# yulong314/multi_camera_calibration

Hardware: AMD Instinct MI355X
Metric: corner residual+Jacobian evals/sec + ms/LM-iter; RMS reproj-err vs ref (higher is better)
Workload: dtype f64; 1 GPU; config4: 4 omnidirectional cameras, 1000 synthetic 11x8-board views (BASELINE.json configs[3]), one Gauss-Newton step per 'step'; model=omnidirectional, cameras=4, views=1000, edges=3958, params=6018, parallelism=photo-sharded x1, transport=none, state_dtype=f32, jacobian_dtype=f64

## Files before the change

multi_camera_calibration_amd/csrc/mcc_api.cpp:

```cpp
#include <hip/hip_runtime.h>
#include <rccl/rccl.h>

#include <algorithm>
#include <chrono>
#include <cmath>
#include <cstdio>
#include <cstring>
#include <mutex>
#include <numeric>
#include <string>
#include <vector>

#include "../../include/mcc.h"
#include "mcc_internal.h"

using mcc::State;

namespace {

thread_local std::string g_err;

int fail(int code, const std::string& msg) {
    g_err = msg;
    return code;
// ... 99 lines not shown
void tilt_matrix(double tx, double ty, double M[9]) {
    const double cx = std::cos(tx), sx = std::sin(tx), cy = std::cos(ty), sy = std::sin(ty);
    const double rx[9] = {1, 0, 0, 0, cx, sx, 0, -sx, cx};
    const double ry[9] = {cy, 0, -sy, 0, 1, 0, sy, 0, cy};
    double rxy[9];
    for (int i = 0; i < 3; ++i)
        for (int j = 0; j < 3; ++j) {
            double s = 0;
            for (int k = 0; k < 3; ++k) s += ry[3 * i + k] * rx[3 * k + j];
            rxy[3 * i + j] = s;
        }
    const double pz[9] = {rxy[8], 0, -rxy[2], 0, rxy[8], -rxy[5], 0, 0, 1};
    for (int i = 0; i < 3; ++i)
        for (int j = 0; j < 3; ++j) {
            double s = 0;
            for (int k = 0; k < 3; ++k) s += pz[3 * i + k] * rxy[3 * k + j];
            M[3 * i + j] = s;
        }
}

}

struct mcc_problem {
    int model = 0, C = 0, V = 0, E = 0, nd = 0, m = 0, P = 0, device = 0;
    long long corners = 0;
    bool rational = false;
    int prism = 0;
    int has_back = 0;
    int max_epp = 1, nblk = 0, n_items = 0, n_pairs = 0, n_norm_chunks = 0;
    size_t n_pair_doubles = 0;
    int n_pgroups = 0, max_gpairs = 0, max_gcon = 0, max_gedges = 0;
    size_t photo_shmem = 0;
    int use_group = 1;
    size_t group_shmem = 0;
    int group_lanes = 32;
    static constexpr int kFusedMaxM = 30;
    int fused = 0, group_size = 1, n_groups = 1;
    int max_cpp = 1;
    hipStream_t stream = nullptr;

    std::vector<int> dev2ref_edge;
    std::vector<long long> dev2ref_corner;
    std::vector<int> edge_n_dev;

    DevBuf<float> obj_x, obj_y, obj_z, img_u, img_v, x, xerr, K, D, xi, cam_rt, cam_pose, resid, edge_sum, corner_err;
    DevBuf<long long> stamps;
    DevBuf<double> ds_rt, Y, pairprod, zp, gp_tot, item_out, packed, dg, delta, photo_norm, alpha, contrib, gsum, W;
    DevBuf<double> erec, echain, eh;
    DevBuf<double> tilt;
    DevBuf<double> ssinv;
    DevBuf<int> ssinv_ok;
    DevBuf<int> photo_ptr, photo_corner, edge_gblock, block_items, edge_photo, counter, cnt, cnt_blk;
    DevBuf<int> pgrp_ptr, pgrp_edge, gpair_ptr, gcon_ptr;
    DevBuf<int> prep_ptr, prep_edge;
    bool poison = false;
    int poison_level = 0;
    bool peer_push = true;
    int schur_one_level = 0;
    int n_prep = 0, prep_lanes = 1;
    bool warm = false;
    hipStream_t side = nullptr;
    double* sinv = nullptr;
    double* prev2 = nullptr;
    int prev_stride = 0;
    unsigned* wsync = nullptr;
    double* xsol = nullptr;
    bool helper_refine = false;
    int helper_early = 0;
    int inv_la = 0;
    DevBuf<long long> warm_stats;
    int warm_poison = 0;
    long long warm_wait_ticks = 1000000000LL, warm_idle_ticks = 4000000000LL, warm_delay_ticks = 0;
    long long spare_delay_ticks = 0;
    bool small_stats = false;
    bool gfold = false;
    int fold_direct = 0;
    int fold_dyn = 0;
    int fold_first = 0;
    DevBuf<int> fold_ticket;
    int max_item_slots = 0;
    DevBuf<double> fnorm, fiv;
    int fault_photo = -1;
    DevBuf<unsigned char> edge_lphoto;
    DevBuf<unsigned> gcon;
    DevBuf<int4> edge_info, items, gpairs;
    DevBuf<State> state;
    State* h_state = nullptr;
    float* h_x = nullptr;
    int packed_len = 0, ntri = 0;

    static constexpr int kGraphSteps = 8;
    static constexpr int kGraphSizes = 7;
    hipGraphExec_t gexec[kGraphSizes] = {};
    hipGraphExec_t lin_graph = nullptr;
    int lin_graph_n = 0;
    DevBuf<float> xsave;
    DevBuf<double> ysave, zpsave;
    int graph_sizes = kGraphSizes;
    bool use_graph = true;
    bool stepping = false;

    ncclComm_t comm = nullptr;
    int nranks = 1, rank = 0;

    static constexpr int kPeerMaxRanks = MCC_PEER_MAX_RANKS;
    unsigned long long* inbox = nullptr;
// ... 37 lines not shown
                        p->helper_refine && !copy_prev ? 1 : 0, p->xsol, p->helper_early,
                        p->stamps.p ? p->stamps.p + p->stamps.n - 64 : nullptr, p->inv_la};
}

mcc::PeerCtx peer_ctx(mcc_problem* p, bool on) {
    mcc::PeerCtx pc{};
    if (!on) return pc;
    pc.inbox = p->inbox;
    pc.peers = p->peers_dev;
    pc.nranks = p->peer_n;
    pc.rank = p->rank;
    pc.Lc = p->packed_len;
    pc.timeout = p->peer_timeout;
    return pc;
}

void drop_graphs(mcc_problem* p) {
    for (auto& g : p->gexec)
        if (g) { (void)hipGraphExecDestroy(g); g = nullptr; }
    if (p->lin_graph) { (void)hipGraphExecDestroy(p->lin_graph); p->lin_graph = nullptr; }
}

int enqueue_step(mcc_problem* p, int do_update, float* resid_dev, bool lin_only = false) {
    using namespace mcc;
    const bool tim = p->timing && p->ev_used + 2 <= (int)p->ev_lin.size();
    const bool swarm = p->ssinv.p && (p->peer_on || !p->comm);
    if (p->poison) {
        for (auto* b : {&p->contrib, &p->gsum, &p->item_out, &p->pairprod, &p->packed, &p->ssinv})
            if (b->p && b->n && !(swarm && b == &p->packed) && !(p->fused && b == &p->ssinv))
                HIPCHK(hipMemsetAsync(b->p, 0xFF, sizeof(double) * b->n, p->stream));
        if (swarm && !p->fused) HIPCHK(hipMemsetAsync(p->ssinv_ok.p, 0xFF, 2 * sizeof(int), p->stream));
        for (auto* b : {&p->erec, &p->echain, &p->eh})
            if (b->p && b->n) HIPCHK(hipMemsetAsync(b->p, 0xFF, sizeof(double) * b->n, p->stream));
        if (p->poison_level > 1 && p->dg.p) HIPCHK(hipMemsetAsync(p->dg.p, 0xFF, sizeof(double) * p->dg.n, p->stream));
    }
    if (tim) HIPCHK(hipEventRecord(p->ev_step[p->ev_used], p->stream));
    if (tim) HIPCHK(hipEventRecord(p->ev_lin[p->ev_used], p->stream));
    LinArgs la{};
    la.state = p->state.p;
    la.photo_ptr = p->photo_ptr.p;
    la.photo_corner = p->photo_corner.p;
    la.max_cpp = p->max_cpp;
    la.edge_info = p->edge_info.p;
    la.obj_x = p->obj_x.p; la.obj_y = p->obj_y.p; la.obj_z = p->obj_z.p;
    la.img_u = p->img_u.p; la.img_v = p->img_v.p;
    la.x = p->x.p;
    la.K = p->K.p; la.D = p->D.p; la.xi = p->xi.p; la.tilt = p->tilt.p;
    la.cam_rt = p->cam_rt.p; la.ds_rt = p->ds_rt.p;
    la.nd = p->nd; la.global_dim = p->m;
    la.n_cams = p->C; la.has_back = p->has_back;
    la.Y = p->Y.p; la.zp = p->zp.p;
    la.pgrp_ptr = p->pgrp_ptr.p; la.pgrp_edge = p->pgrp_edge.p; la.edge_lphoto = p->edge_lphoto.p; la.gpair_ptr = p->gpair_ptr.p; la.gpairs = p->gpairs.p;
    la.gcon_ptr = p->gcon_ptr.p; la.gcon = p->gcon.p; la.pairprod = p->pairprod.p;
    la.prep_ptr = p->prep_ptr.p; la.prep_edge = p->prep_edge.p; la.n_prep = p->n_prep; la.prep_lanes = p->prep_lanes;
    la.n_pgroups = p->n_pgroups; la.max_gpairs = p->max_gpairs; la.max_gcon = p->max_gcon; la.max_gedges = p->max_gedges;
    la.gp_tot = p->gp_tot.p;
    la.resid = resid_dev;
    la.gblock = p->edge_gblock.p;
    la.dg = p->dg.p;
    la.photo_norm = p->photo_norm.p;
    la.stamps = p->stamps.p;
    la.fault_photo = p->fault_photo;
    const bool lwarm = swarm && (do_update || !p->fused);
    la.ssinv = lwarm ? p->ssinv.p : nullptr;
    la.ssinv_ok = lwarm ? p->ssinv_ok.p : nullptr;
    la.spare_wait = p->warm_wait_ticks;
    la.spare_delay = p->spare_delay_ticks;
    const bool peer = p->peer_on;
    const bool rccl = p->comm != nullptr && !peer;
    la.fused = p->fused;
    la.group_size = p->group_size; la.n_groups = p->n_groups;
    la.rank = p->rank; la.fuse_solve = rccl ? 0 : 1;
    la.peer = peer_ctx(p, peer && p->fused);
    la.contrib = p->contrib.p; la.gsum = p->gsum.p; la.cnt = p->cnt.p; la.packed = p->packed.p; la.W = p->W.p;
    la.solve = solve_ctx(p, do_update);
    la.solve.stamps = nullptr;
    la.n_edges = p->E; la.n_photos = p->V;
    la.erec = p->erec.p; la.echain = p->echain.p; la.eh = p->eh.p;
    SchurArgs sa{};
    const bool split = rccl || p->m > 30;
    if (!p->fused) {
        sa.state = p->state.p;
        sa.items = p->items.p;
        sa.pairprod = p->pairprod.p;
        sa.item_out = p->item_out.p;
        sa.n_items = p->n_items;
        sa.photo_norm = p->photo_norm.p; sa.n_photos = p->V;
        sa.counter = p->counter.p;
        sa.cnt_blk = p->cnt_blk.p;
        sa.nblk = p->nblk;
        sa.block_items = p->block_items.p;
        sa.packed = p->packed.p;
        sa.m = p->m; sa.rank = p->rank; sa.fuse_solve = split ? 0 : 1;
        sa.one_level = p->schur_one_level;
        sa.prev2 = p->warm && do_update && !p->comm && !p->peer_on ? p->prev2 : nullptr;
        sa.prev_stride = p->prev_stride;
        sa.wpub = sa.prev2 && p->helper_refine ? p->wsync : nullptr;
        sa.wpub_early = p->helper_early;
        sa.ssinv = swarm ? p->ssinv.p : nullptr;
        sa.ssinv_ok = swarm ? p->ssinv_ok.p : nullptr;
        sa.peer = peer_ctx(p, peer && !split);
        sa.solve = solve_ctx(p, do_update);
        sa.stamps = p->stamps.p ? p->stamps.p + mcc::kStampStride * (size_t)std::max(p->V, 1) : nullptr;
    }
    const bool fold = p->gfold && !lin_only;
    if (fold) {
// ... 493 lines not shown
    p->group_size = std::max(1, (int)std::ceil(std::sqrt((double)std::max(V, 1))));
    p->n_groups = (std::max(V, 1) + p->group_size - 1) / p->group_size;

    std::vector<float> cam_rt(6 * C, 0.f);
    if (d->model == MCC_MODEL_DOUBLESIDE) {
        for (int c = 0; c < C; ++c) {
            double R[9], r[3];
            for (int i = 0; i < 3; ++i)
                for (int j = 0; j < 3; ++j) R[i * 3 + j] = d->cam_pose[16 * c + i * 4 + j];
            host_rodrigues_m2v(R, r);
            for (int i = 0; i < 3; ++i) { cam_rt[6 * c + i] = (float)r[i]; cam_rt[6 * c + 3 + i] = d->cam_pose[16 * c + i * 4 + 3]; }
        }
    }
    double ds_rt[6] = {0, 0, 0, 0, 0, 0};
    if (d->ds_pose && d->model == MCC_MODEL_PINHOLE) {
        double R[9];
        for (int i = 0; i < 3; ++i)
            for (int j = 0; j < 3; ++j) R[i * 3 + j] = d->ds_pose[i * 4 + j];
        host_rodrigues_m2v(R, ds_rt);
        for (int i = 0; i < 3; ++i) ds_rt[3 + i] = d->ds_pose[i * 4 + 3];
    }
    std::vector<double> alpha(4096);
    for (size_t k = 0; k < alpha.size(); ++k) alpha[k] = std::pow(0.95, (double)k + 1.0);

    HIPC(p->obj_x.upload(ox.data(), ncorner)); HIPC(p->obj_y.upload(oy.data(), ncorner));
    HIPC(p->obj_z.upload(oz.data(), ncorner));
    HIPC(p->img_u.upload(iu.data(), ncorner)); HIPC(p->img_v.upload(iv.data(), ncorner));
    HIPC(p->edge_info.upload(info.data(), E));
    HIPC(p->edge_gblock.upload(gblock.data(), E));
    HIPC(p->edge_photo.upload(ephoto.data(), E));
    HIPC(p->photo_ptr.upload(photo_ptr.data(), V + 1));
    HIPC(p->photo_corner.upload(photo_corner.data(), V + 1));
    HIPC(p->K.upload(d->K, 9 * C));
    HIPC(p->D.upload(d->D, (size_t)d->nd * C));
    std::vector<float> xi(C, 0.f);
    if (d->xi) std::copy(d->xi, d->xi + C, xi.begin());
    HIPC(p->xi.upload(xi.data(), C));
    HIPC(p->cam_rt.upload(cam_rt.data(), 6 * C));
    std::vector<float> cp(16 * C, 0.f);
    if (d->cam_pose) std::copy(d->cam_pose, d->cam_pose + 16 * C, cp.begin());
    HIPC(p->cam_pose.upload(cp.data(), 16 * C));
    HIPC(p->ds_rt.upload(ds_rt, 6));
    HIPC(p->alpha.upload(alpha.data(), alpha.size()));
    HIPC(p->pgrp_ptr.upload(pgrp_ptr.data(), pgrp_ptr.size()));
    {
        std::vector<int> pgrp_edge(pgrp_ptr.size());
        for (size_t g = 0; g < pgrp_ptr.size(); ++g) pgrp_edge[g] = photo_ptr[pgrp_ptr[g]];
        HIPC(p->pgrp_edge.upload(pgrp_edge.data(), pgrp_edge.size()));
        std::vector<unsigned char> lph(std::max(E, 1), 0);
        for (size_t g = 0; g + 1 < pgrp_ptr.size(); ++g)
            for (int v = pgrp_ptr[g]; v < pgrp_ptr[g + 1]; ++v)
                for (int e = photo_ptr[v]; e < photo_ptr[v + 1]; ++e) lph[e] = (unsigned char)(v - pgrp_ptr[g]);
        HIPC(p->edge_lphoto.upload(lph.data(), lph.size()));
    }
    if (!p->fused && !p->use_group) {
        if (const char* f = std::getenv("MCC_PREP_LANES")) p->prep_lanes = std::atoi(f) == 4 ? 4 : 1;
        std::vector<int> pp(1, 0);
        for (int v = 0; v < V;) {
            int w = v, edges = 0;
            while (w < V && w - v < mcc::kPrepPhotos &&
                   (w == v || edges + (photo_ptr[w + 1] - photo_ptr[w]) <= mcc::kPrepEdges)) {
                edges += photo_ptr[w + 1] - photo_ptr[w];
                ++w;
            }
            pp.push_back(w);
            v = w;
        }
        std::vector<int> pe(pp.size());
        for (size_t g = 0; g < pp.size(); ++g) pe[g] = photo_ptr[pp[g]];
        p->n_prep = (int)pp.size() - 1;
        HIPC(p->prep_ptr.upload(pp.data(), pp.size()));
        HIPC(p->prep_edge.upload(pe.data(), pe.size()));
    }
    HIPC(p->gpair_ptr.upload(gpair_ptr.data(), gpair_ptr.size()));
    HIPC(p->gpairs.upload(gpairs.data(), gpairs.size()));
    HIPC(p->gcon_ptr.upload(gcon_ptr.data(), gcon_ptr.size()));
    HIPC(p->gcon.upload(gcon.data(), gcon.size()));
    HIPC(p->items.upload(items.data(), items.size()));
    HIPC(p->block_items.upload(block_items.data(), block_items.size()));
    HIPC(p->x.alloc(p->P)); HIPC(p->xerr.alloc(p->P));
    HIPC(p->Y.alloc(36 * (size_t)E));
    HIPC(p->pairprod.alloc(p->fused ? 0 : p->n_pair_doubles));
    const bool use_split = !p->fused && !p->use_group;
    HIPC(p->erec.alloc(use_split ? 12 * (size_t)E : 0));
    HIPC(p->echain.alloc(use_split ? 54 * (size_t)E : 0));
    HIPC(p->eh.alloc(use_split ? 90 * (size_t)E : 0));
    HIPC(p->zp.alloc(6 * (size_t)V));
    HIPC(p->gp_tot.alloc(6 * (size_t)V));
    HIPC(p->item_out.alloc(48 * (size_t)(items.size() + p->n_norm_chunks + 24)));
    HIPC(hipMemset(p->item_out.p, 0, sizeof(double) * p->item_out.n));
    HIPC(p->counter.alloc(1));
    HIPC(hipMemset(p->counter.p, 0, sizeof(int)));
    HIPC(p->cnt_blk.alloc(p->nblk));
    HIPC(hipMemset(p->cnt_blk.p, 0, sizeof(int) * std::max(p->nblk, 1)));
    p->ntri = p->m * (p->m + 1) / 2;
    p->packed_len = p->ntri + 2 * p->m + 2;
    HIPC(p->packed.alloc(p->packed_len));
    HIPC(p->dg.alloc(p->m)); HIPC(p->delta.alloc(p->P));
    HIPC(p->photo_norm.alloc(2 * (size_t)V));
    if (p->fused) {
        const size_t lcp = (size_t)((p->packed_len + 1) & ~1);
        HIPC(p->contrib.alloc(lcp * std::max(V, 1)));
        HIPC(p->gsum.alloc(lcp * p->n_groups));
        HIPC(p->W.alloc((size_t)6 * p->m * std::max(V, 1)));
        HIPC(p->cnt.alloc(p->n_groups + 1));
        HIPC(hipMemset(p->cnt.p, 0, sizeof(int) * (p->n_groups + 1)));
// ... 82 lines not shown
        HIPC(hipMalloc((void**)&p->sinv, M * M * sizeof(double)));
        p->prev_stride = (p->ntri + p->m + 1) & ~1;
        HIPC(hipExtMallocWithFlags((void**)&p->prev2, 2 * (size_t)p->prev_stride * sizeof(double), hipDeviceMallocUncached));
        if (int r = reset_prev2(p, true)) return bail(r);
        HIPC(hipExtMallocWithFlags((void**)&p->wsync, 8 * sizeof(unsigned), hipDeviceMallocUncached));
        HIPC(hipMemset(p->wsync, 0, 8 * sizeof(unsigned)));
        HIPC(hipExtMallocWithFlags((void**)&p->xsol, 128 * sizeof(double), hipDeviceMallocUncached));
        HIPC(hipMemset(p->xsol, 0, 128 * sizeof(double)));
        if (!p->warm_stats.p) HIPC(p->warm_stats.alloc(5));
        HIPC(hipMemset(p->warm_stats.p, 0, 5 * sizeof(long long)));
        HIPC(stream_pool().take(d->device, &p->side, true));
    }
#undef HIPC
    (void)rc;
    *out = p;
    return MCC_OK;
}

void mcc_destroy(mcc_problem* p) {
    if (!p) return;
    (void)hipSetDevice(p->device);
    const bool side_drained = p->side && hipStreamSynchronize(p->side) == hipSuccess;
    const bool drained = p->stream && hipStreamSynchronize(p->stream) == hipSuccess;
    if (p->sinv) (void)hipFree(p->sinv);
    if (p->prev2) (void)hipFree(p->prev2);
    if (p->wsync) (void)hipFree(p->wsync);
    if (p->xsol) (void)hipFree(p->xsol);
    p->warm_stats.release();
    drop_graphs(p);
    p->xsave.release(); p->ysave.release(); p->zpsave.release();
    for (auto e : p->ev_lin) (void)hipEventDestroy(e);
    for (auto e : p->ev_step) (void)hipEventDestroy(e);
    for (auto e : p->ev_opt) if (e) (void)hipEventDestroy(e);
    for (auto e : p->ev_x) (void)hipEventDestroy(e);
    for (auto e : p->ev_marks) (void)hipEventDestroy(e);
    for (auto e : p->ev_win) if (e) (void)hipEventDestroy(e);
    if (p->comm) (void)ncclCommDestroy(p->comm);
    for (void* m : p->peer_mapped) (void)hipIpcCloseMemHandle(m);
    if (p->peers_dev) (void)hipFree(p->peers_dev);
    if (p->peer_scratch) (void)hipFree(p->peer_scratch);
    if (p->inbox) (void)hipFree(p->inbox);
    p->obj_x.release(); p->obj_y.release(); p->obj_z.release(); p->img_u.release(); p->img_v.release();
    p->x.release(); p->xerr.release(); p->K.release(); p->D.release(); p->xi.release(); p->cam_rt.release();
    p->cam_pose.release(); p->resid.release(); p->edge_sum.release(); p->corner_err.release(); p->stamps.release();
    p->contrib.release(); p->gsum.release(); p->cnt.release(); p->W.release();
    p->ds_rt.release(); p->Y.release(); p->pairprod.release(); p->zp.release();
    p->erec.release(); p->echain.release(); p->eh.release(); p->tilt.release(); p->fnorm.release(); p->fiv.release();
    p->fold_ticket.release(); p->ssinv.release(); p->ssinv_ok.release();
    p->gp_tot.release(); p->item_out.release(); p->packed.release(); p->dg.release(); p->delta.release();
    p->photo_norm.release(); p->alpha.release();
    p->photo_ptr.release(); p->photo_corner.release(); p->edge_gblock.release(); p->block_items.release(); p->counter.release(); p->cnt_blk.release();
    p->edge_photo.release(); p->edge_info.release(); p->items.release(); p->gpairs.release();
    p->prep_ptr.release(); p->prep_edge.release();
    p->pgrp_ptr.release(); p->pgrp_edge.release(); p->edge_lphoto.release(); p->gpair_ptr.release(); p->gcon_ptr.release(); p->gcon.release();
    p->state.release();
    if (p->h_state) (void)hipHostFree(p->h_state);
    if (p->h_x) (void)hipHostFree(p->h_x);
    if (drained) stream_pool().give(p->device, p->stream);
    else if (p->stream) (void)hipStreamDestroy(p->stream);
    if (side_drained) stream_pool().give(p->device, p->side, true);
    else if (p->side) (void)hipStreamDestroy(p->side);
    delete p;
}

int mcc_set_params(mcc_problem* p, const float* x, int n) {
    if (!p || !x || n != p->P) return fail(MCC_EINVAL, "mcc_set_params: size mismatch");
    HIPCHK(hipSetDevice(p->device));
    HIPCHK(hipStreamSynchronize(p->stream));
    HIPCHK(hipMemcpy(p->x.p, x, sizeof(float) * n, hipMemcpyHostToDevice));
    int rc = set_state(p, 1, 0, 0, 0.0);
    if (rc) return rc;
    const int zero = 0;
    HIPCHK(hipMemcpy(&p->state.p->pending, &zero, sizeof(int), hipMemcpyHostToDevice));
    return MCC_OK;
}

int mcc_get_params(mcc_problem* p, float* x, int n) {
    if (!p || !x || n != p->P) return fail(MCC_EINVAL, "mcc_get_params: size mismatch");
    HIPCHK(hipSetDevice(p->device));
    int rc = flush_pending(p);
    if (rc) return rc;
    HIPCHK(hipStreamSynchronize(p->stream));
    HIPCHK(hipMemcpy(x, p->x.p, sizeof(float) * n, hipMemcpyDeviceToHost));
    return MCC_OK;
}

int mcc_linearize_solve(mcc_problem* p, double* delta, double* jte) {
    if (!p) return fail(MCC_EINVAL, "null problem");
    HIPCHK(hipSetDevice(p->device));
    int rc = flush_pending(p);
    if (rc) return rc;
    if ((rc = set_state(p, 0, 0, 0, 0.0))) return rc;
    if ((rc = enqueue_step(p, 0, nullptr))) return rc;
    if ((rc = enqueue_backsub(p, 0))) return rc;
    if ((rc = read_state(p))) return rc;
    if ((rc = check_state_error(p))) return rc;
    if (delta) HIPCHK(hipMemcpy(delta, p->delta.p, sizeof(double) * p->P, hipMemcpyDeviceToHost));
    if (jte) {
        std::vector<double> pk(p->packed_len), gp(6 * (size_t)p->V);
        HIPCHK(hipMemcpy(pk.data(), p->packed.p, sizeof(double) * p->packed_len, hipMemcpyDeviceToHost));
        if (p->V) HIPCHK(hipMemcpy(gp.data(), p->gp_tot.p, sizeof(double) * 6 * p->V, hipMemcpyDeviceToHost));
        for (int i = 0; i < p->m; ++i) jte[i] = pk[p->ntri + p->m + i];
        for (int i = 0; i < 6 * p->V; ++i) jte[p->m + i] = gp[i];
    }
    return MCC_OK;
}
// ... 584 lines not shown
```

multi_camera_calibration_amd/csrc/mcc_group.hpp:

```cpp


template <int MODEL, bool BACK, int L, int GW = 28>
__device__ __forceinline__ void group_prologue(const double* ph, const double* ct, const double* sds, int side,
                                               int sub, double* S, double* P, double* Gb) {
    const double* R1 = ph;
    const double* Jr1 = ph + 9;
    const double* T1 = ph + 18;
    const double* R2 = ct;
    const double* Jl2 = ct + 9;
    const double* T2 = ct + 18;
    double* X = S;
    double* W = S + 15;
    for (int e = sub; e < 12; e += L) {
        if (e < 9) {
            const int i = e / 3, j = e % 3;
            X[e] = dot3_nc(R2[i * 3], R1[j], R2[i * 3 + 1], R1[3 + j], R2[i * 3 + 2], R1[6 + j]);
        } else {
            const int i = e - 9;
            const double q = dot3_nc(R2[i * 3], T1[0], R2[i * 3 + 1], T1[1], R2[i * 3 + 2], T1[2]);
            X[12 + i] = q;
            X[9 + i] = add_nc(q, T2[i]);
        }
    }
    wave_sync_lds();
// ... 552 lines not shown
        fold_final_reset(la, src, have, useiv);
        return;
    }
    __syncthreads();
    if (a.peer.nranks > 0) {
        if (!peer_exchange(a.peer, st, a.packed)) {
            fold_final_reset(la, src, have, useiv);
            return;
        }
        for (int t = tid; t < ntri + m; t += nt) {
            const double v = a.packed[t];
            if (t < ntri) {
                int i, j;
                packed_ij(t, m, i, j);
                S[i * m + j] = v;
                S[j * m + i] = v;
            } else {
                r[t - ntri] = v;
            }
        }
        if (tid < 2) norms[tid] = a.packed[ntri + 2 * m + tid];
        __syncthreads();
    }
    SSTAMP(srow, 3, 0);
    SolveCtx sc = a.solve;
    sc.stamps = srow;
    solve_global<false>(sc, S, r, norms[0], norms[1], nullptr, ivok ? Iv : nullptr);
    SSTAMP(srow, 7, 0);
    fold_final_reset(la, src, have, useiv);
}
template <int NT>
__device__ __forceinline__ void fold_final(const LinArgs& la) {
    if (NT == 512 && la.fold_direct) {
        fold_final_direct(la);
        return;
    }
    constexpr int UM = kSchurOneLevelLoads * 256 / NT;
    const int n = 48 * la.fold_parts + (la.fsa.ssinv != nullptr ? la.fsa.m * la.fsa.m + 1 : 0);
    if (n <= UM / 2 * NT) fold_final_u<UM / 2>(la);
    else fold_final_u<UM>(la);
}

#ifndef MCC_GROUP_PAIR_THREADS
#define MCC_GROUP_PAIR_THREADS 256
#endif
#ifndef MCC_GROUP_OCC
#define MCC_GROUP_OCC 2
#endif
template <int MODEL, bool RATIONAL, int PRISM, bool BACK, int L>
__device__ __forceinline__ bool group_body(const LinArgs& a, const int grp) {
    constexpr int NT = kGroupRound * L, EPW = 64 / L;
    State* st = a.state;
    const int tid = threadIdx.x, lane = tid & 63, wave = tid >> 6;
    const int done = st->done, pending = st->pending;
    const double alpha_prev = st->alpha;
    const int p0 = a.pgrp_ptr[grp], np = a.pgrp_ptr[grp + 1] - p0;
    const int ge0 = a.pgrp_edge[grp], gne = a.pgrp_edge[grp + 1] - ge0;
    const int q0 = a.gpair_ptr[grp], nq = a.gpair_ptr[grp + 1] - q0;
    const int c0 = a.gcon_ptr[grp], nc = a.gcon_ptr[grp + 1] - c0;
    if (done) return false;
    long long* stp = a.stamps ? a.stamps + kStampStride * (size_t)grp : nullptr;
    SSTAMP(stp, 0, 0);
    const int C = a.n_cams, m = a.global_dim;
    extern __shared__ __attribute__((aligned(16))) double smem[];
    const GroupLayout GL = group_layout(gne, C, nq, nc);
    double* rec = smem + GL.rec;
    double* s27 = smem + GL.s27;
    double* sLi = smem + GL.sLi;
    double* sv = smem + GL.sv;
    double* sph = smem + GL.sph;
    double* sxn = smem + GL.sxn;
    double* spart = smem + GL.spart;
    double* sdg = smem + GL.sdg;
    double* ctab = smem + GL.ctab;
    double* ktab = smem + GL.ktab;
    double* sds = smem + GL.sds;
    double* sP = smem + GL.sP;
    double* sGb = smem + GL.sGb;
    int* ibase = reinterpret_cast<int*>(smem + GL.ndoubles);
    int4* sInfo = reinterpret_cast<int4*>(ibase + GL.iInfo);
    int* sgb = ibase + GL.iGb;
    int* seq = ibase + GL.iEq;
    int* sph0 = ibase + GL.iPh;
    int4* spq = reinterpret_cast<int4*>(ibase + GL.iPq);
    unsigned* scn = reinterpret_cast<unsigned*>(ibase + GL.iCn);
    float(*sC)[kGChunk][EPW] = reinterpret_cast<float(*)[kGChunk][EPW]>(smem + GL.sU + wave * (5 * kGChunk * EPW / 2));
    GroupChain* sCH = reinterpret_cast<GroupChain*>(smem + GL.sU + wave * (5 * kGChunk * EPW / 2));
    static_assert(EPW * sizeof(GroupChain) <= 5 * kGChunk * EPW * sizeof(float), "k_group chain union");

    const int g = lane % EPW, sub = lane / EPW;
    auto stage = [&](int eoff, int cc0, int cn) {
        constexpr int PER = kGChunk / L;
        float v[PER][5];
        int sb = sub;
        asm volatile("" : "+v"(sb));
#pragma unroll
        for (int u = 0; u < PER; ++u) {
            const int i = sb + L * u;
            const unsigned c = (unsigned)(eoff + cc0 + (i < cn ? i : 0));
            v[u][0] = a.obj_x[c];
            v[u][1] = a.obj_y[c];
            v[u][2] = a.obj_z[c];
            v[u][3] = a.img_u[c];
            v[u][4] = a.img_v[c];
        }
#pragma unroll
        for (int u = 0; u < PER; ++u) {
            const int i = sb + L * u;
            if (i < cn) {
#pragma unroll
                for (int f = 0; f < 5; ++f) sC[f][i][g] = v[u][f];
            }
        }
    };

    constexpr int CAM0 = NT / 2, DST = CAM0 + 63;
    double om2[3] = {0.0, 0.0, 0.0}, T2[3] = {0.0, 0.0, 0.0};
    {
        {
            const int le = wave * EPW + g;
            const int4 info = le < gne ? a.edge_info[ge0 + le] : make_int4(0, 0, 0, 0);
            if (le < gne) stage(info.z, 0, min(info.w, kGChunk));
        }
        for (int t = tid; t < gne; t += NT) {
            sInfo[t] = a.edge_info[ge0 + t];
            sgb[t] = a.gblock[ge0 + t];
            seq[t] = a.edge_lphoto[ge0 + t];
        }
        if (tid <= np) sph0[tid] = a.photo_ptr[p0 + tid] - ge0;
        for (int t = tid; t < nq; t += NT) spq[t] = a.gpairs[q0 + t];
        for (int t = tid; t < nc; t += NT) scn[t] = a.gcon[c0 + t];
        for (int t = tid; t < m; t += NT) sdg[t] = a.dg[t];
        if (tid >= CAM0 && tid < CAM0 + C) {
            const int c = tid - CAM0;
            if (MODEL == MCC_MODEL_DOUBLESIDE) {
#pragma unroll
                for (int k = 0; k < 3; ++k) { om2[k] = a.cam_rt[6 * c + k]; T2[k] = a.cam_rt[6 * c + 3 + k]; }
            } else if (c == 0) {
#pragma unroll
                for (int k = 0; k < 3; ++k) { om2[k] = 0.0; T2[k] = 0.0; }
            } else {
#pragma unroll
                for (int k = 0; k < 3; ++k) { om2[k] = a.x[6 * (c - 1) + k]; T2[k] = a.x[6 * (c - 1) + 3 + k]; }
            }
            double* kt = ktab + kGIntr * c;
            const float* Kc = a.K + 9 * c;
            kt[0] = Kc[0]; kt[1] = Kc[4]; kt[2] = Kc[2]; kt[3] = Kc[5]; kt[4] = Kc[1];
            kt[5] = MODEL == MCC_MODEL_OMNI ? (double)a.xi[c] : 0.0;
            const int nd = a.nd;
#pragma unroll
            for (int q = 0; q < 12; ++q) kt[6 + q] = q < nd ? (double)a.D[nd * c + q] : 0.0;
            if (PRISM == 2)
#pragma unroll
                for (int q = 0; q < 9; ++q) kt[18 + q] = a.tilt[9 * c + q];
        } else if (BACK && tid == DST) {
            if (MODEL == MCC_MODEL_DOUBLESIDE) {
#pragma unroll
                for (int k = 0; k < 3; ++k) { om2[k] = a.x[k]; T2[k] = a.x[3 + k]; }
            } else {
#pragma unroll
                for (int k = 0; k < 3; ++k) { om2[k] = a.ds_rt[k]; T2[k] = a.ds_rt[3 + k]; }
            }
        }
    }
    float xo = 0.f;
    double zk = 0.0;
    const int pq = (tid - 192) / 6, pk = (tid - 192) % 6;
    const bool ptask = tid >= 192 && pq < np;
    double2 pn0 = make_double2(0.0, 0.0);
    if (ptask) {
        xo = a.x[m + 6 * (size_t)(p0 + pq) + pk];
        if (pending) zk = a.zp[6 * (size_t)(p0 + pq) + pk];
        else if (a.fold && pk == 0) pn0 = *reinterpret_cast<const double2*>(a.photo_norm + 2 * (size_t)(p0 + pq));
    }
    double y0[6];
    int gb0 = -1;
    if (pending && tid < 6 * gne) {
        const int le = tid / 6, k = tid % 6;
        gb0 = a.gblock[ge0 + le];
        const double* Ye = a.Y + 36 * (size_t)(ge0 + le);
#pragma unroll
        for (int i = 0; i < 6; ++i) y0[i] = Ye[6 * i + k];
    }
    __syncthreads();
    SSTAMP(stp, 1, 0);
    if (pending) {
        for (int t = tid; t < 6 * gne; t += NT) {
            const int le = t / 6, k = t % 6;
            int gbl = gb0;
            double y[6];
            if (t == tid) {
#pragma unroll
                for (int i = 0; i < 6; ++i) y[i] = y0[i];
            } else {
                gbl = sgb[le];
                const double* Ye = a.Y + 36 * (size_t)(ge0 + le);
#pragma unroll
                for (int i = 0; i < 6; ++i) y[i] = Ye[6 * i + k];
            }
            const double* d = sdg + 6 * (gbl < 0 ? 0 : gbl);
            double sk = 0.0;
#pragma unroll
            for (int i = 0; i < 6; ++i) sk += y[i] * d[i];
            spart[6 * le + k] = gbl < 0 ? 0.0 : sk;
        }
    }
    __syncthreads();
    if (tid >= CAM0 && tid < CAM0 + C) {
        const int c = tid - CAM0;
        Rot r2;
        rodrigues_v2m(om2, r2);
        double J[9];
        so3_jac(om2, r2, +1.0, J);
        double* ct = ctab + 24 * c;
#pragma unroll
        for (int k = 0; k < 9; ++k) { ct[k] = r2.R[k]; ct[9 + k] = J[k]; }
#pragma unroll
        for (int k = 0; k < 3; ++k) ct[18 + k] = T2[k];
    } else if (BACK && tid == DST) {
        Rot rd;
        rodrigues_v2m(om2, rd);
        double J[9];
        so3_jac(om2, rd, -1.0, J);
#pragma unroll
        for (int k = 0; k < 9; ++k) { sds[k] = rd.R[k]; sds[9 + k] = J[k]; }
#pragma unroll
        for (int k = 0; k < 3; ++k) sds[18 + k] = T2[k];
    }
    if (ptask) {
        float xn = xo;
        double Gk = 0.0;
        if (pending) {
            double t = zk;
            for (int le = sph0[pq]; le < sph0[pq + 1]; ++le) t -= spart[6 * le + pk];
            const float G = (float)(alpha_prev * t);
            xn = xo + G;
            a.x[m + 6 * (size_t)(p0 + pq) + pk] = xn;
            Gk = (double)G;
        }
        sxn[16 * pq + pk] = (double)xn;
        sxn[16 * pq + 8 + pk] = Gk;
    }
    wave_sync_lds();
    if (ptask && pk == 0) {
        const double* xs = sxn + 16 * pq;
        if (pending) {
            double g2 = 0.0, x2 = 0.0;
#pragma unroll
            for (int q = 0; q < 6; ++q) {
                g2 += xs[8 + q] * xs[8 + q];
                x2 += xs[q] * xs[q];
            }
            a.photo_norm[2 * (size_t)(p0 + pq)] = g2;
            a.photo_norm[2 * (size_t)(p0 + pq) + 1] = x2;
            pn0 = make_double2(g2, x2);
        }
        if (a.fold) {
            sxn[16 * pq + 6] = pn0.x;
            sxn[16 * pq + 7] = pn0.y;
        }
        const double om1[3] = {xs[0], xs[1], xs[2]};
        Rot r1;
        rodrigues_v2m(om1, r1);
        double* ph = sph + 24 * pq;
        so3_jac(om1, r1, -1.0, ph + 9);
#pragma unroll
        for (int k = 0; k < 9; ++k) ph[k] = r1.R[k];
#pragma unroll
        for (int k = 0; k < 3; ++k) ph[18 + k] = xs[3 + k];
    }
    __syncthreads();
    SSTAMP(stp, 2, 0);

    for (int rb = 0; rb < gne; rb += kGroupRound) {
        const int es = wave * EPW + g, le = rb + es;
        const bool ev = le < gne;
        const int4 info = ev ? sInfo[le] : make_int4(0, 0, 0, 0);
        const int cam = info.x;
        double* P = sP + kGRecP * es;
        double* Gbe = sGb + 56 * es;
        if (rb > 0 && ev) stage(info.z, 0, min(info.w, kGChunk));
        if (ev) {
            group_prologue<MODEL, BACK, L>(sph + 24 * seq[le], ctab + 24 * cam, sds, info.y, sub, rec + kGRec * le, P, Gbe);
            const double* kt = ktab + kGIntr * cam;
            for (int k = sub; k < (PRISM == 2 ? 27 : 18); k += L) P[12 + k] = kt[k];
        }
        wave_sync_lds();
        if (rb == 0) SSTAMP(stp, 3, 0);
        double acc[32];
#pragma unroll
        for (int q = 0; q < 32; ++q) acc[q] = 0.0;
        const int nn = info.w;
        for (int cc0 = 0;; cc0 += kGChunk) {
            if (cc0 >= nn) break;
            const int cn = min(nn - cc0, kGChunk);
            if (cc0 > 0) {
                wave_sync_lds();
                stage(info.z, cc0, cn);
                wave_sync_lds();
            }
#pragma unroll 1
            for (int i = sub; i < cn; i += L) {
                int po = 0;
                asm volatile("" : "+v"(po));
                const double* Pq = P + po;
                double R[9], T[3], kd[12];
#pragma unroll
                for (int q = 0; q < 9; ++q) R[q] = Pq[q];
#pragma unroll
                for (int q = 0; q < 3; ++q) T[q] = Pq[9 + q];
#pragma unroll
                for (int q = 0; q < 12; ++q) kd[q] = Pq[18 + q];
                const double fx = Pq[12], fy = Pq[13], cx = Pq[14], cy = Pq[15], sk = Pq[16], xi = Pq[17];
                const double X = sC[0][i][g], Y = sC[1][i][g], Z = sC[2][i][g];
                const float ou = sC[3][i][g], ov = sC[4][i][g];
                double Yr[3], D[6];
                float u, v;
                if (MODEL == MCC_MODEL_OMNI)
                    omni_corner(R, T, kd, fx, fy, cx, cy, sk, xi, X, Y, Z, Yr, u, v, D);
                else
                    pinhole_corner<RATIONAL, PRISM>(R, T, kd, fx, fy, cx, cy, X, Y, Z, Yr, u, v, D, Pq + 30);
                const float euf = ou - u, evf = ov - v;
                if (a.resid) {
                    const size_t c = (size_t)info.z + cc0 + i;
                    a.resid[2 * c] = euf;
// ... 439 lines not shown
```

multi_camera_calibration_amd/csrc/mcc_internal.h:

```cpp
#pragma once
#include <hip/hip_runtime.h>

#include "../../include/mcc.h"

namespace mcc {

constexpr int kStampStride = 32;
constexpr int kSchurStampStride = 16;

struct State {
    int iter;
    int done;
    int crit_type;
    int max_count;
    double eps;
    double change;
    double alpha;
    double cam_normG2, cam_normX2;
    int error;
    int pending;
    unsigned int epoch;
    long long xchg_ticks;
    unsigned int spare_ack;
};
// ... 54 lines not shown
    const int4* edge_info;
    const float* obj_x; const float* obj_y; const float* obj_z;
    const float* img_u; const float* img_v;
    float* x;
    const float* K; const float* D; const float* xi;
    const double* tilt;
    const float* cam_rt;
    const double* ds_rt;
    int nd, global_dim, n_cams, has_back;
    double* Y;
    const int* pgrp_ptr;
    const int* pgrp_edge;
    const unsigned char* edge_lphoto;
    const int* gpair_ptr;
    const int4* gpairs;
    const int* gcon_ptr;
    const unsigned* gcon;
    double* pairprod;
    int n_pgroups, max_gpairs, max_gcon, max_gedges;
    double* zp;
    double* gp_tot;
    float* resid;
    const int* gblock;
    const double* dg;
    double* photo_norm;
    long long* stamps;
    int fused, group_size, n_groups, rank, fuse_solve;
    double* contrib;
    double* gsum;
    int* cnt;
    double* packed;
    double* W;
    SolveCtx solve;
    PeerCtx peer;
    int n_edges, n_photos;
    double* erec;
    double* echain;
    double* eh;
    const int* prep_ptr;
    const int* prep_edge;
    int n_prep, prep_lanes;
    int fault_photo;
    int fold_first;
    double* ssinv;
    int* ssinv_ok;
    long long spare_wait, spare_delay;
    int fold, fold_parts;
    int fold_direct;
    int fold_dyn;
    int* fold_ticket;
    SchurArgs fsa;
    double* fnorm;
    double* fiv;
};
constexpr long long kFoldEmpty = -1LL;

constexpr int kItemSingle = 256;
constexpr int kPhotoGroup = 8;
constexpr int kPhotoGroupEdges = 64;
constexpr int kGroupRound = 16;
__host__ __device__ inline size_t photo_lds_doubles(int gne) {
    return (size_t)64 * gne + (size_t)70 * kPhotoGroup;
}
__host__ __device__ inline size_t photo_lds_bytes(int gne, int npairs, int ncon) {
    return photo_lds_doubles(gne) * 8 + 4 * (size_t)((2 * gne + 3) & ~3) + 16 * (size_t)npairs + 4 * (size_t)ncon;
}

constexpr int kGChunk = 96;
constexpr int kGIntr = 28;
constexpr int kGRecP = 40;
constexpr int kGRec = 92;

struct GroupLayout {
    int rec, s27, sLi, sv, sph, sxn, spart, sdg, ctab, ktab, sds, sP, sGb, sU, ndoubles;
    int iInfo, iGb, iEq, iPh, iPq, iCn, nints;
};
__host__ __device__ inline GroupLayout group_layout(int gne, int C, int nq, int nc) {
    GroupLayout L;
    L.rec = 0;
    L.s27 = L.rec + kGRec * gne;
    L.sLi = L.s27 + 28 * kPhotoGroup;
    L.sv = L.sLi + 36 * kPhotoGroup;
    L.sph = L.sv + 6 * kPhotoGroup;
    L.sxn = L.sph + 24 * kPhotoGroup;
    L.spart = L.sxn + 16 * kPhotoGroup;
    L.sdg = L.spart + 6 * gne;
    L.ctab = L.sdg + 128;
    L.ktab = L.ctab + 24 * C;
    L.sds = L.ktab + kGIntr * C;
    L.sP = L.sds + 32;
    L.sGb = L.sP + kGRecP * kGroupRound;
    L.sU = L.sGb + 56 * kGroupRound;
    L.ndoubles = L.sU + 4 * (5 * kGChunk * 4 / 2);
    L.ndoubles = (L.ndoubles + 1) & ~1;
    L.iInfo = 0;
    L.iGb = L.iInfo + 4 * gne;
    L.iEq = L.iGb + gne;
    L.iPh = L.iEq + gne;
    L.iPq = (L.iPh + kPhotoGroup + 1 + 3) & ~3;
    L.iCn = L.iPq + 4 * nq;
    L.nints = L.iCn + nc;
    return L;
}
__host__ __device__ inline size_t group_lds_bytes(int gne, int C, int nq, int nc) {
    const GroupLayout L = group_layout(gne, C, nq, nc);
    return (size_t)L.ndoubles * 8 + (size_t)L.nints * 4;
}

constexpr int kPrepEdges = 16;
constexpr int kPrepPhotos = kPhotoGroup;
struct PrepLayout {
    int tab, S, sdg, sxn, scam, ndoubles;
    int iInfo, iGb, iPh, nints;
// ... 109 lines not shown
```

Measured before the change: 13.04 billion corner evals/s.

## Pack per-group headers and camera intrinsics on host, batch group-kernel prologue loads

Precomputes a per-group header (ranges, photo offsets, first-round edge info, gblock and local-photo indices) and a per-camera intrinsics table on the host at setup. The group linearization kernel then reads these through wave-uniform, predicated register loads instead of chains of dependent scattered loads. Those loads are issued together with the first corner-chunk staging load, and the LDS store of that chunk is deferred until after the pending-update phase so its latency overlaps other work. This shortens the kernel prologue latency, at the cost of extra setup buffers, more register pressure, and intrinsics that are frozen at setup time.

New measurement: 13.74 billion corner evals/s, median of 6. 1.05x the previous value.

```diff
diff --git a/multi_camera_calibration_amd/csrc/mcc_api.cpp b/multi_camera_calibration_amd/csrc/mcc_api.cpp
--- a/multi_camera_calibration_amd/csrc/mcc_api.cpp
+++ b/multi_camera_calibration_amd/csrc/mcc_api.cpp
@@ -175,6 +175,8 @@
     DevBuf<int> ssinv_ok;
     DevBuf<int> photo_ptr, photo_corner, edge_gblock, block_items, edge_photo, counter, cnt, cnt_blk;
     DevBuf<int> pgrp_ptr, pgrp_edge, gpair_ptr, gcon_ptr;
+    DevBuf<int> ghdr;
+    DevBuf<double> kintr;
     DevBuf<int> prep_ptr, prep_edge;
     bool poison = false;
     int poison_level = 0;
@@ -318,6 +320,7 @@
     la.Y = p->Y.p; la.zp = p->zp.p;
     la.pgrp_ptr = p->pgrp_ptr.p; la.pgrp_edge = p->pgrp_edge.p; la.edge_lphoto = p->edge_lphoto.p; la.gpair_ptr = p->gpair_ptr.p; la.gpairs = p->gpairs.p;
     la.gcon_ptr = p->gcon_ptr.p; la.gcon = p->gcon.p; la.pairprod = p->pairprod.p;
+    la.ghdr = p->ghdr.p; la.kintr = p->kintr.p;
     la.prep_ptr = p->prep_ptr.p; la.prep_edge = p->prep_edge.p; la.n_prep = p->n_prep; la.prep_lanes = p->prep_lanes;
     la.n_pgroups = p->n_pgroups; la.max_gpairs = p->max_gpairs; la.max_gcon = p->max_gcon; la.max_gedges = p->max_gedges;
     la.gp_tot = p->gp_tot.p;
@@ -917,6 +920,33 @@
             for (int v = pgrp_ptr[g]; v < pgrp_ptr[g + 1]; ++v)
                 for (int e = photo_ptr[v]; e < photo_ptr[v + 1]; ++e) lph[e] = (unsigned char)(v - pgrp_ptr[g]);
         HIPC(p->edge_lphoto.upload(lph.data(), lph.size()));
+        std::vector<int> hdr((size_t)mcc::kGHdrInts * std::max(NG, 1), 0);
+        for (int g = 0; g < NG; ++g) {
+            int* h = hdr.data() + (size_t)mcc::kGHdrInts * g;
+            const int p0 = pgrp_ptr[g], np = pgrp_ptr[g + 1] - p0, ge0 = photo_ptr[p0], gne = photo_ptr[p0 + np] - ge0;
+            h[0] = p0; h[1] = np; h[2] = ge0; h[3] = gne;
+            h[4] = gpair_ptr[g]; h[5] = gpair_ptr[g + 1] - gpair_ptr[g];
+            h[6] = gcon_ptr[g]; h[7] = gcon_ptr[g + 1] - gcon_ptr[g];
+            for (int q = 0; q <= mcc::kPhotoGroup; ++q) h[mcc::kGHdrPhoto + q] = photo_ptr[p0 + std::min(q, np)] - ge0;
+            for (int le = 0; le < std::min(gne, mcc::kGroupRound); ++le) {
+                const int4 f = info[ge0 + le];
+                int* hi = h + mcc::kGHdrInfo + 4 * le;
+                hi[0] = f.x; hi[1] = f.y; hi[2] = f.z; hi[3] = f.w;
+                h[mcc::kGHdrGb + le] = gblock[ge0 + le];
+                h[mcc::kGHdrEq + le] = lph[ge0 + le];
+            }
+        }
+        HIPC(p->ghdr.upload(hdr.data(), hdr.size()));
+        std::vector<double> kin((size_t)mcc::kGIntr * C, 0.0);
+        for (int c = 0; c < C; ++c) {
+            double* kt = kin.data() + (size_t)mcc::kGIntr * c;
+            const float* Kc = d->K + 9 * c;
+            kt[0] = Kc[0]; kt[1] = Kc[4]; kt[2] = Kc[2]; kt[3] = Kc[5]; kt[4] = Kc[1];
+            kt[5] = d->model == MCC_MODEL_OMNI ? (double)xi[c] : 0.0;
+            for (int q = 0; q < 12; ++q) kt[6 + q] = q < d->nd ? (double)d->D[d->nd * c + q] : 0.0;
+            if (p->prism == 2) tilt_matrix(d->D[14 * c + 12], d->D[14 * c + 13], kt + 18);
+        }
+        HIPC(p->kintr.upload(kin.data(), kin.size()));
     }
     if (!p->fused && !p->use_group) {
         if (const char* f = std::getenv("MCC_PREP_LANES")) p->prep_lanes = std::atoi(f) == 4 ? 4 : 1;
@@ -1105,6 +1135,7 @@
     p->photo_ptr.release(); p->photo_corner.release(); p->edge_gblock.release(); p->block_items.release(); p->counter.release(); p->cnt_blk.release();
     p->edge_photo.release(); p->edge_info.release(); p->items.release(); p->gpairs.release();
     p->prep_ptr.release(); p->prep_edge.release();
+    p->ghdr.release(); p->kintr.release();
     p->pgrp_ptr.release(); p->pgrp_edge.release(); p->edge_lphoto.release(); p->gpair_ptr.release(); p->gcon_ptr.release(); p->gcon.release();
     p->state.release();
     if (p->h_state) (void)hipHostFree(p->h_state);
diff --git a/multi_camera_calibration_amd/csrc/mcc_group.hpp b/multi_camera_calibration_amd/csrc/mcc_group.hpp
--- a/multi_camera_calibration_amd/csrc/mcc_group.hpp
+++ b/multi_camera_calibration_amd/csrc/mcc_group.hpp
@@ -628,12 +628,14 @@
     constexpr int NT = kGroupRound * L, EPW = 64 / L;
     State* st = a.state;
     const int tid = threadIdx.x, lane = tid & 63, wave = tid >> 6;
+    const int wv = __builtin_amdgcn_readfirstlane(wave);
+    const int* __restrict__ hdr = a.ghdr + (size_t)kGHdrInts * grp;
     const int done = st->done, pending = st->pending;
     const double alpha_prev = st->alpha;
-    const int p0 = a.pgrp_ptr[grp], np = a.pgrp_ptr[grp + 1] - p0;
-    const int ge0 = a.pgrp_edge[grp], gne = a.pgrp_edge[grp + 1] - ge0;
-    const int q0 = a.gpair_ptr[grp], nq = a.gpair_ptr[grp + 1] - q0;
-    const int c0 = a.gcon_ptr[grp], nc = a.gcon_ptr[grp + 1] - c0;
+    const int p0 = hdr[kGHdrRange], np = hdr[kGHdrRange + 1];
+    const int ge0 = hdr[kGHdrRange + 2], gne = hdr[kGHdrRange + 3];
+    const int q0 = hdr[kGHdrRange + 4], nq = hdr[kGHdrRange + 5];
+    const int c0 = hdr[kGHdrRange + 6], nc = hdr[kGHdrRange + 7];
     if (done) return false;
     long long* stp = a.stamps ? a.stamps + kStampStride * (size_t)grp : nullptr;
     SSTAMP(stp, 0, 0);
@@ -665,11 +667,8 @@
     static_assert(EPW * sizeof(GroupChain) <= 5 * kGChunk * EPW * sizeof(float), "k_group chain union");
 
     const int g = lane % EPW, sub = lane / EPW;
-    auto stage = [&](int eoff, int cc0, int cn) {
-        constexpr int PER = kGChunk / L;
-        float v[PER][5];
-        int sb = sub;
-        asm volatile("" : "+v"(sb));
+    constexpr int PER = kGChunk / L;
+    auto stage_load = [&](float (&v)[PER][5], int sb, int eoff, int cc0, int cn) {
 #pragma unroll
         for (int u = 0; u < PER; ++u) {
             const int i = sb + L * u;
@@ -680,6 +679,8 @@
             v[u][3] = a.img_u[c];
             v[u][4] = a.img_v[c];
         }
+    };
+    auto stage_store = [&](const float (&v)[PER][5], int sb, int cn) {
 #pragma unroll
         for (int u = 0; u < PER; ++u) {
             const int i = sb + L * u;
@@ -688,55 +689,46 @@
                 for (int f = 0; f < 5; ++f) sC[f][i][g] = v[u][f];
             }
         }
+    };
+    auto stage = [&](int eoff, int cc0, int cn) {
+        float v[PER][5];
+        int sb = sub;
+        asm volatile("" : "+v"(sb));
+        stage_load(v, sb, eoff, cc0, cn);
+        stage_store(v, sb, cn);
     };
 
     constexpr int CAM0 = NT / 2, DST = CAM0 + 63;
     double om2[3] = {0.0, 0.0, 0.0}, T2[3] = {0.0, 0.0, 0.0};
-    {
-        {
-            const int le = wave * EPW + g;
-            const int4 info = le < gne ? a.edge_info[ge0 + le] : make_int4(0, 0, 0, 0);
-            if (le < gne) stage(info.z, 0, min(info.w, kGChunk));
-        }
-        for (int t = tid; t < gne; t += NT) {
-            sInfo[t] = a.edge_info[ge0 + t];
-            sgb[t] = a.gblock[ge0 + t];
-            seq[t] = a.edge_lphoto[ge0 + t];
-        }
-        if (tid <= np) sph0[tid] = a.photo_ptr[p0 + tid] - ge0;
-        for (int t = tid; t < nq; t += NT) spq[t] = a.gpairs[q0 + t];
-        for (int t = tid; t < nc; t += NT) scn[t] = a.gcon[c0 + t];
-        for (int t = tid; t < m; t += NT) sdg[t] = a.dg[t];
-        if (tid >= CAM0 && tid < CAM0 + C) {
-            const int c = tid - CAM0;
-            if (MODEL == MCC_MODEL_DOUBLESIDE) {
-#pragma unroll
-                for (int k = 0; k < 3; ++k) { om2[k] = a.cam_rt[6 * c + k]; T2[k] = a.cam_rt[6 * c + 3 + k]; }
-            } else if (c == 0) {
-#pragma unroll
-                for (int k = 0; k < 3; ++k) { om2[k] = 0.0; T2[k] = 0.0; }
-            } else {
-#pragma unroll
-                for (int k = 0; k < 3; ++k) { om2[k] = a.x[6 * (c - 1) + k]; T2[k] = a.x[6 * (c - 1) + 3 + k]; }
-            }
-            double* kt = ktab + kGIntr * c;
-            const float* Kc = a.K + 9 * c;
-            kt[0] = Kc[0]; kt[1] = Kc[4]; kt[2] = Kc[2]; kt[3] = Kc[5]; kt[4] = Kc[1];
-            kt[5] = MODEL == MCC_MODEL_OMNI ? (double)a.xi[c] : 0.0;
-            const int nd = a.nd;
-#pragma unroll
-            for (int q = 0; q < 12; ++q) kt[6 + q] = q < nd ? (double)a.D[nd * c + q] : 0.0;
-            if (PRISM == 2)
-#pragma unroll
-                for (int q = 0; q < 9; ++q) kt[18 + q] = a.tilt[9 * c + q];
-        } else if (BACK && tid == DST) {
-            if (MODEL == MCC_MODEL_DOUBLESIDE) {
-#pragma unroll
-                for (int k = 0; k < 3; ++k) { om2[k] = a.x[k]; T2[k] = a.x[3 + k]; }
-            } else {
-#pragma unroll
-                for (int k = 0; k < 3; ++k) { om2[k] = a.ds_rt[k]; T2[k] = a.ds_rt[3 + k]; }
-            }
+    const int le0 = wave * EPW + g;
+    const int4 info0 = *reinterpret_cast<const int4*>(hdr + kGHdrInfo + 4 * le0);
+    int4 rInfo = make_int4(0, 0, 0, 0);
+    int rGb = 0, rEq = 0, rPh = 0;
+    if (wv == 0) {
+        const int t = lane < kGroupRound ? lane : 0;
+        rInfo = *reinterpret_cast<const int4*>(hdr + kGHdrInfo + 4 * t);
+        rGb = hdr[kGHdrGb + t];
+        rEq = hdr[kGHdrEq + t];
+        rPh = hdr[kGHdrPhoto + (lane <= kPhotoGroup ? lane : 0)];
+    }
+    int4 rPq = make_int4(0, 0, 0, 0);
+    unsigned rCn = 0;
+    double rDg = 0.0, rKt = 0.0;
+    if (wv * 64 < nq) rPq = a.gpairs[q0 + (tid < nq ? tid : 0)];
+    if (wv * 64 < nc) rCn = a.gcon[c0 + (tid < nc ? tid : 0)];
+    if (wv * 64 < m) rDg = a.dg[tid < m ? tid : 0];
+    if (wv * 64 < kGIntr * C) rKt = a.kintr[tid < kGIntr * C ? tid : 0];
+    float rCam[6] = {0.f, 0.f, 0.f, 0.f, 0.f, 0.f};
+    double rDs[6] = {0.0, 0.0, 0.0, 0.0, 0.0, 0.0};
+    if (wv == CAM0 / 64) {
+        const int c = lane < C ? lane : 0;
+        const float* src = MODEL == MCC_MODEL_DOUBLESIDE ? a.cam_rt + 6 * c : a.x + 6 * (c > 0 ? c - 1 : 0);
+        if (BACK && MODEL == MCC_MODEL_DOUBLESIDE) src = tid == DST ? a.x : src;
+#pragma unroll
+        for (int k = 0; k < 6; ++k) rCam[k] = src[k];
+        if (BACK && MODEL != MCC_MODEL_DOUBLESIDE) {
+#pragma unroll
+            for (int k = 0; k < 6; ++k) rDs[k] = a.ds_rt[k];
         }
     }
     float xo = 0.f;
@@ -744,20 +736,69 @@
     const int pq = (tid - 192) / 6, pk = (tid - 192) % 6;
     const bool ptask = tid >= 192 && pq < np;
     double2 pn0 = make_double2(0.0, 0.0);
-    if (ptask) {
-        xo = a.x[m + 6 * (size_t)(p0 + pq) + pk];
-        if (pending) zk = a.zp[6 * (size_t)(p0 + pq) + pk];
-        else if (a.fold && pk == 0) pn0 = *reinterpret_cast<const double2*>(a.photo_norm + 2 * (size_t)(p0 + pq));
-    }
-    double y0[6];
+    if (wv == 3) {
+        const size_t pi = ptask ? 6 * (size_t)(p0 + pq) + pk : 0;
+        xo = a.x[m + pi];
+        if (pending) zk = a.zp[pi];
+        else if (a.fold) pn0 = *reinterpret_cast<const double2*>(a.photo_norm + (ptask && pk == 0 ? 2 * (size_t)(p0 + pq) : 0));
+    }
+    double y0[6] = {0.0, 0.0, 0.0, 0.0, 0.0, 0.0};
     int gb0 = -1;
-    if (pending && tid < 6 * gne) {
-        const int le = tid / 6, k = tid % 6;
+    if (pending && wv * 64 < 6 * gne) {
+        const bool act = tid < 6 * gne;
+        const int le = act ? tid / 6 : 0, k = act ? tid % 6 : 0;
         gb0 = a.gblock[ge0 + le];
         const double* Ye = a.Y + 36 * (size_t)(ge0 + le);
 #pragma unroll
         for (int i = 0; i < 6; ++i) y0[i] = Ye[6 * i + k];
     }
+    float cv0[PER][5];
+    int sb0 = sub;
+    asm volatile("" : "+v"(sb0));
+    const int cn0 = min(info0.w, kGChunk);
+    __builtin_amdgcn_sched_barrier(0);
+    stage_load(cv0, sb0, info0.z, 0, cn0);
+    __builtin_amdgcn_sched_barrier(0);
+#pragma unroll
+    for (int k = 0; k < 6; ++k) asm volatile("" : "+v"(rCam[k]));
+    if (wv == 0) {
+        if (lane < kGroupRound && lane < gne) {
+            sInfo[lane] = rInfo;
+            sgb[lane] = rGb;
+            seq[lane] = rEq;
+        }
+        if (lane <= np) sph0[lane] = rPh;
+    }
+    if (tid < nq) spq[tid] = rPq;
+    if (tid < nc) scn[tid] = rCn;
+    if (tid < m) sdg[tid] = rDg;
+    if (tid < kGIntr * C) ktab[tid] = rKt;
+    if (tid >= CAM0 && tid < CAM0 + C) {
+        const bool fixed0 = MODEL != MCC_MODEL_DOUBLESIDE && tid == CAM0;
+#pragma unroll
+        for (int k = 0; k < 3; ++k) {
+            om2[k] = fixed0 ? 0.0 : (double)rCam[k];
+            T2[k] = fixed0 ? 0.0 : (double)rCam[3 + k];
+        }
+    } else if (BACK && tid == DST) {
+#pragma unroll
+        for (int k = 0; k < 3; ++k) {
+            om2[k] = MODEL == MCC_MODEL_DOUBLESIDE ? (double)rCam[k] : rDs[k];
+            T2[k] = MODEL == MCC_MODEL_DOUBLESIDE ? (double)rCam[3 + k] : rDs[3 + k];
+        }
+    }
+#pragma unroll 1
+    for (int t = kGroupRound + tid; t < gne; t += NT) {
+        sInfo[t] = a.edge_info[ge0 + t];
+        sgb[t] = a.gblock[ge0 + t];
+        seq[t] = a.edge_lphoto[ge0 + t];
+    }
+#pragma unroll 1
+    for (int t = NT + tid; t < nq; t += NT) spq[t] = a.gpairs[q0 + t];
+#pragma unroll 1
+    for (int t = NT + tid; t < nc; t += NT) scn[t] = a.gcon[c0 + t];
+#pragma unroll 1
+    for (int t = NT + tid; t < kGIntr * C; t += NT) ktab[t] = a.kintr[t];
     __syncthreads();
     SSTAMP(stp, 1, 0);
     if (pending) {
@@ -847,6 +888,7 @@
     }
     __syncthreads();
     SSTAMP(stp, 2, 0);
+    stage_store(cv0, sb0, cn0);
 
     for (int rb = 0; rb < gne; rb += kGroupRound) {
         const int es = wave * EPW + g, le = rb + es;
diff --git a/multi_camera_calibration_amd/csrc/mcc_internal.h b/multi_camera_calibration_amd/csrc/mcc_internal.h
--- a/multi_camera_calibration_amd/csrc/mcc_internal.h
+++ b/multi_camera_calibration_amd/csrc/mcc_internal.h
@@ -130,13 +130,24 @@
     SchurArgs fsa;
     double* fnorm;
     double* fiv;
-};
+    const int* ghdr;
+    const double* kintr;
+};
+constexpr int kGHdrRange = 0;
+constexpr int kGHdrPhoto = 8;
+constexpr int kGHdrInfo = 20;
+constexpr int kGHdrGb = 84;
+constexpr int kGHdrEq = 100;
+constexpr int kGHdrInts = 128;
 constexpr long long kFoldEmpty = -1LL;
 
 constexpr int kItemSingle = 256;
 constexpr int kPhotoGroup = 8;
 constexpr int kPhotoGroupEdges = 64;
 constexpr int kGroupRound = 16;
+static_assert(kGHdrPhoto + kPhotoGroup + 1 <= kGHdrInfo && kGHdrInfo % 4 == 0 && kGHdrInfo + 4 * kGroupRound == kGHdrGb &&
+                  kGHdrGb + kGroupRound == kGHdrEq && kGHdrEq + kGroupRound <= kGHdrInts,
+              "k_group header layout");
 __host__ __device__ inline size_t photo_lds_doubles(int gne) {
     return (size_t)64 * gne + (size_t)70 * kPhotoGroup;
 }
```
